# MicahZoltu/lodestar

Measured on AMD Instinct MI355X. Metric: verified signature sets/sec (mainnet attestation mix), higher is better.
Workload: dtype u32 (381-bit Montgomery; device products on 14x28-bit limbs); 1 GPU; c3: gossip attestation flood, 6 slot(s) per batch, 7 batches in flight per GPU; slots_per_batch=6, sets_per_gpu=116736, jobs_per_gpu=104448, pubkeys_per_gpu=1683456, parallelism=dp1 (sets sharded), exchange=False, inflight=7, world_size_seen=1, pubkeys=indices into the GPU-resident table, signing_roots_per_gpu=6918

## Files before the change

lodestar_amd/csrc/lb_consts.h:

```cpp
#pragma once
#include "lb_common.h"

#define LB_PINV 0xfffcfffdu
#define LB_X_ABS 0xd201000000010000ull
#define LB_PINV28 0xffcfffdu
#define LB_P28_0 0xfffaaabu
#define LB_P28_1 0xfefffffu
#define LB_P28_2 0x3ffffb9u
#define LB_P28_3 0xfffeb15u
#define LB_P28_4 0x6241eabu
#define LB_P28_5 0xa0f6b0fu
#define LB_P28_6 0xf6730d2u
#define LB_P28_7 0xf38512bu
#define LB_P28_8 0x4774b84u
#define LB_P28_9 0x4bacd76u
#define LB_P28_10 0xba7b643u
#define LB_P28_11 0xe69a4b1u
#define LB_P28_12 0x1ea397fu
#define LB_P28_13 0x001a011u
#define LB_P0 0xffffaaabu
#define LB_P1 0xb9feffffu
#define LB_P2 0xb153ffffu
#define LB_P3 0x1eabfffeu
#define LB_P4 0xf6b0f624u
#define LB_P5 0x6730d2a0u
#define LB_P6 0xf38512bfu
#define LB_P7 0x64774b84u
#define LB_P8 0x434bacd7u
#define LB_P9 0x4b1ba7b6u
#define LB_P10 0x397fe69au
#define LB_P11 0x1a0111eau
LB_CONST uint32_t LB_P[12] = {0xffffaaab, 0xb9feffff, 0xb153ffff, 0x1eabfffe, 0xf6b0f624, 0x6730d2a0, 0xf38512bf, 0x64774b84, 0x434bacd7, 0x4b1ba7b6, 0x397fe69a, 0x1a0111ea};
LB_CONST uint32_t LB_ONE[12] = {0x0002fffd, 0x76090000, 0xc40c0002, 0xebf4000b, 0x53c758ba, 0x5f489857, 0x70525745, 0x77ce5853, 0xa256ec6d, 0x5c071a97, 0xfa80e493, 0x15f65ec3};
LB_CONST uint32_t LB_R2[12] = {0x1c341746, 0xf4df1f34, 0x09d104f1, 0x0a76e6a6, 0x4c95b6d5, 0x8de5476c, 0x939d83c0, 0x67eb88a9, 0xb519952d, 0x9a793e85, 0x92cae3aa, 0x11988fe5};
LB_CONST uint32_t LB_2P256[12] = {0xc5ce820f, 0x075b3cd7, 0x1c3edb0b, 0x3ec6ba62, 0x2bff6bce, 0x168a13d8, 0xf8c449d2, 0x87663c4b, 0xddc8d830, 0x15f34c83, 0x9caa2e85, 0x0f9628b4};
LB_CONST uint32_t LB_B1[12] = {0x000cfff3, 0xaa270000, 0xfc34000a, 0x53cc0032, 0x6b0a807f, 0x478fe97a, 0xe6ba24d7, 0xb1d37ebe, 0xbf78ab2f, 0x8ec9733b, 0x3d83de7e, 0x09d64551};
LB_CONST uint32_t LB_B1_3[12] = {0x0027552e, 0x44760000, 0x43480020, 0xdcb8009a, 0x4a6e8b59, 0x6f7ee9ce, 0xc0a95bc6, 0xb10330b7, 0xfb1e54b7, 0x6140b1fc, 0x7f0bb4e1, 0x0381be09};
LB_CONST uint32_t LB_B2[24] = {0x000cfff3, 0xaa270000, 0xfc34000a, 0x53cc0032, 0x6b0a807f, 0x478fe97a, 0xe6ba24d7, 0xb1d37ebe, 0xbf78ab2f, 0x8ec9733b, 0x3d83de7e, 0x09d64551, 0x000cfff3, 0xaa270000, 0xfc34000a, 0x53cc0032, 0x6b0a807f, 0x478fe97a, 0xe6ba24d7, 0xb1d37ebe, 0xbf78ab2f, 0x8ec9733b, 0x3d83de7e, 0x09d64551};
LB_CONST uint32_t LB_B2_3[24] = {0x0027552e, 0x44760000, 0x43480020, 0xdcb8009a, 0x4a6e8b59, 0x6f7ee9ce, 0xc0a95bc6, 0xb10330b7, 0xfb1e54b7, 0x6140b1fc, 0x7f0bb4e1, 0x0381be09, 0x0027552e, 0x44760000, 0x43480020, 0xdcb8009a, 0x4a6e8b59, 0x6f7ee9ce, 0xc0a95bc6, 0xb10330b7, 0xfb1e54b7, 0x6140b1fc, 0x7f0bb4e1, 0x0381be09};
LB_CONST uint32_t LB_EXP_PM2[12] = {0xffffaaa9, 0xb9feffff, 0xb153ffff, 0x1eabfffe, 0xf6b0f624, 0x6730d2a0, 0xf38512bf, 0x64774b84, 0x434bacd7, 0x4b1ba7b6, 0x397fe69a, 0x1a0111ea};
LB_CONST uint32_t LB_EXP_SQRT[12] = {0xffffeaab, 0xee7fbfff, 0xac54ffff, 0x07aaffff, 0x3dac3d89, 0xd9cc34a8, 0x3ce144af, 0xd91dd2e1, 0x90d2eb35, 0x92c6e9ed, 0x8e5ff9a6, 0x0680447a};
LB_CONST uint32_t LB_EXP_ISQRT[12] = {0xffffeaaa, 0xee7fbfff, 0xac54ffff, 0x07aaffff, 0x3dac3d89, 0xd9cc34a8, 0x3ce144af, 0xd91dd2e1, 0x90d2eb35, 0x92c6e9ed, 0x8e5ff9a6, 0x0680447a};
LB_CONST uint32_t LB_EXP_LEGENDRE[12] = {0xffffd555, 0xdcff7fff, 0x58a9ffff, 0x0f55ffff, 0x7b587b12, 0xb3986950, 0x79c2895f, 0xb23ba5c2, 0x21a5d66b, 0x258dd3db, 0x1cbff34d, 0x0d0088f5};
LB_CONST uint32_t LB_HALF_P[12] = {0xffffd555, 0xdcff7fff, 0x58a9ffff, 0x0f55ffff, 0x7b587b12, 0xb3986950, 0x79c2895f, 0xb23ba5c2, 0x21a5d66b, 0x258dd3db, 0x1cbff34d, 0x0d0088f5};
LB_CONST uint32_t LB_INV2[12] = {0x00015554, 0x18040000, 0x3ab00001, 0x85500005, 0x253c276f, 0x633cb57c, 0x31ebb502, 0x6e22d1ec, 0xf2d14ca2, 0xd3916126, 0x1a006596, 0x17fbb857};
LB_CONST uint32_t LB_R3[12] = {0xd94ca1e0, 0xed48ac6b, 0x03a7adf8, 0x315f831e, 0x615e29dd, 0x9a53352a, 0x921e1761, 0x34c04e5e, 0x65724728, 0x2512d435, 0x91755d4d, 0x0aa63460};
LB_CONST uint32_t LB_P_X1[13] = {0xffffaaab, 0xb9feffff, 0xb153ffff, 0x1eabfffe, 0xf6b0f624, 0x6730d2a0, 0xf38512bf, 0x64774b84, 0x434bacd7, 0x4b1ba7b6, 0x397fe69a, 0x1a0111ea, 0x00000000};
LB_CONST uint32_t LB_P_X2[13] = {0xffff5556, 0x73fdffff, 0x62a7ffff, 0x3d57fffd, 0xed61ec48, 0xce61a541, 0xe70a257e, 0xc8ee9709, 0x869759ae, 0x96374f6c, 0x72ffcd34, 0x340223d4, 0x00000000};
LB_CONST uint32_t LB_P_X4[13] = {0xfffeaaac, 0xe7fbffff, 0xc54ffffe, 0x7aaffffa, 0xdac3d890, 0x9cc34a83, 0xce144afd, 0x91dd2e13, 0x0d2eb35d, 0x2c6e9ed9, 0xe5ff9a69, 0x680447a8, 0x00000000};
LB_CONST uint32_t LB_P_X8[13] = {0xfffd5558, 0xcff7ffff, 0x8a9ffffd, 0xf55ffff5, 0xb587b120, 0x39869507, 0x9c2895fb, 0x23ba5c27, 0x1a5d66bb, 0x58dd3db2, 0xcbff34d2, 0xd0088f51, 0x00000000};
LB_CONST uint32_t LB_P_X16[13] = {0xfffaaab0, 0x9fefffff, 0x153ffffb, 0xeabfffeb, 0x6b0f6241, 0x730d2a0f, 0x38512bf6, 0x4774b84f, 0x34bacd76, 0xb1ba7b64, 0x97fe69a4, 0xa0111ea3, 0x00000001};
LB_CONST uint32_t LB_P_X32[13] = {0xfff55560, 0x3fdfffff, 0x2a7ffff7, 0xd57fffd6, 0xd61ec483, 0xe61a541e, 0x70a257ec, 0x8ee9709e, 0x69759aec, 0x6374f6c8, 0x2ffcd349, 0x40223d47, 0x00000003};
// ... 43 lines not shown
```

lodestar_amd/csrc/lb_curve.h:

```cpp
#pragma once
#include "lb_field.h"

template <class F>
struct jac {
  F x, y, z;
};
template <class F>
struct aff {
  F x, y;
};

typedef jac<fp> g1j;
typedef jac<fp2> g2j;
typedef aff<fp> g1a;
typedef aff<fp2> g2a;

template <class T, class S>
LB_HD aff<T> aff_as(const aff<S>& a) {
  return aff<T>{T{a.x}, T{a.y}};
}
template <class T, class S>
LB_HD jac<T> jac_as(const jac<S>& a) {
  return jac<T>{T{a.x}, T{a.y}, T{a.z}};
}
// ... 343 lines not shown
  p.y = fp2_sub(lean2_mul<kInl>(rr, fp2_sub(V, p.x)), YJ);
}

template <bool kInl>
LB_HD void g2_add_lean(g2j& p, const g2j& q) {
  if (jac_is_inf(q)) return;
  if (jac_is_inf(p)) {
    p = q;
    return;
  }
  const fp2 Z1Z1 = lean2_sqr<kInl>(p.z), Z2Z2 = lean2_sqr<kInl>(q.z);
  const fp2 ZZ = fp2_sub(fp2_sub(lean2_sqr<kInl>(fp2_add(p.z, q.z)), Z1Z1), Z2Z2);
  const fp2 U1 = lean2_mul<kInl>(p.x, Z2Z2);
  const fp2 S1 = lean2_mul<kInl>(lean2_mul<kInl>(p.y, q.z), Z2Z2);
  const fp2 H = fp2_sub(lean2_mul<kInl>(q.x, Z1Z1), U1);
  const fp2 rr = fp2_dbl(fp2_sub(lean2_mul<kInl>(lean2_mul<kInl>(q.y, p.z), Z1Z1), S1));
  if (fp2_is_zero(H)) {
    if (fp2_is_zero(rr)) {
      p = q;
      g2_dbl_lean<kInl>(p);
    } else {
      p = jac_infinity<fp2>();
    }
    return;
  }
  p.z = lean2_mul<kInl>(ZZ, H);
  const fp2 I = lean2_sqr<kInl>(fp2_dbl(H));
  const fp2 J = lean2_mul<kInl>(H, I);
  const fp2 V = lean2_mul<kInl>(U1, I);
  p.x = fp2_sub(fp2_sub(lean2_sqr<kInl>(rr), J), fp2_dbl(V));
  p.y = fp2_sub(lean2_mul<kInl>(rr, fp2_sub(V, p.x)), fp2_dbl(lean2_mul<kInl>(S1, J)));
}

LB_HD bool g2_aff_in_subgroup_i(const g2a& a) {
  g2j acc = jac_from_aff(a);
#pragma clang loop unroll(disable)
  for (int i = 62; i >= 0; i--) {
    acc = jac_dbl_i(acc);
    if ((LB_X_ABS >> i) & 1ull) acc = jac_add_aff_i<fp2, true>(acc, a);
  }
  if (jac_is_inf(acc)) return false;
  fp2 z2 = fp2_sqr(acc.z);
  fp2 px = fp2_mul(fp2_conj(a.x), fp2_load(LB_PSI_CX));
  if (!fp2_eq(fp2_mul(px, z2), acc.x)) return false;
  fp2 py = fp2_mul(fp2_conj(a.y), fp2_load(LB_PSI_CY));
  return fp2_eq(fp2_mul(fp2_mul(py, z2), acc.z), fp2_neg(acc.y));
}

LB_NI g2j g2_clear_cofactor(g2j p) {
  g2j t1 = jac_neg(jac_mul_xabs(p));
  g2j t2 = g2_psi(p);
  g2j t3 = g2_psi2(jac_dbl(p));
  t3 = jac_add(t3, jac_neg(t2));
  t2 = jac_add(t1, t2);
  t2 = jac_neg(jac_mul_xabs(t2));
  t3 = jac_add(t3, t2);
  t3 = jac_add(t3, jac_neg(t1));
  return jac_add(t3, jac_neg(p));
}

LB_HD bool g1_aff_on_curve(const g1a& a) {
  return fp_eq(fp_sqr(a.y), fp_add(fp_mul(fp_sqr(a.x), a.x), fp_load(LB_B1)));
}
LB_HD bool g2_aff_on_curve(const g2a& a) {
  return fp2_eq(fp2_sqr(a.y), fp2_add(fp2_mul(fp2_sqr(a.x), a.x), fp2_load(LB_B2)));
}
// ... 1 lines not shown
```

lodestar_amd/csrc/lb_field.h:

```cpp
#pragma once
#include "lb_common.h"
#include "lb_consts.h"

struct fp {
  uint32_t v[12];
};
struct fp2 {
  fp c0, c1;
};
struct fp6 {
  fp2 c0, c1, c2;
};
struct fp12 {
  fp6 c0, c1;
};

LB_HD fp fp_load(const uint32_t* c) {
  fp r;
  LB_UNROLL for (int i = 0; i < 12; i++) r.v[i] = c[i];
  return r;
}
LB_HD fp2 fp2_load(const uint32_t* c) {
  fp2 r;
  r.c0 = fp_load(c);
// ... 231 lines not shown

LB_HD fp lb_tab8(const fp* t, uint32_t k) {
  switch (k) {
    case 0: return t[0];
    case 1: return t[1];
    case 2: return t[2];
    case 3: return t[3];
    case 4: return t[4];
    case 5: return t[5];
    case 6: return t[6];
    default: return t[7];
  }
}
LB_HD fp fp_mul_inl(const fp& a, const fp& b) {
#if defined(__HIP_DEVICE_COMPILE__)
  __builtin_amdgcn_sched_barrier(0);
  const fp r = fp_mul28(a, b);
  __builtin_amdgcn_sched_barrier(0);
  return r;
#else
  return fp_mul(a, b);
#endif
}
LB_HD fp fp_sqr_inl(const fp& a) {
#if defined(__HIP_DEVICE_COMPILE__)
  __builtin_amdgcn_sched_barrier(0);
  const fp r = fp_sqr28(a);
  __builtin_amdgcn_sched_barrier(0);
  return r;
#else
  return fp_sqr(a);
#endif
}
struct fp28 {
  uint32_t l[14];
};
LB_HD fp28 fp28_mul_raw(const fp28& a, const fp28& b) {
  const uint32_t P28[14] = {LB_P28_0, LB_P28_1, LB_P28_2, LB_P28_3, LB_P28_4,  LB_P28_5,  LB_P28_6,
                            LB_P28_7, LB_P28_8, LB_P28_9, LB_P28_10, LB_P28_11, LB_P28_12, LB_P28_13};
  uint64_t acc[28];
  LB_UNROLL for (int k = 0; k < 28; k++) acc[k] = 0;
  LB_UNROLL for (int i = 0; i < 14; i++) {
    LB_UNROLL for (int j = 0; j < 14; j++) acc[i + j] += (uint64_t)a.l[i] * b.l[j];
    const uint32_t m = ((uint32_t)acc[i] * LB_PINV28) & 0x0fffffffu;
    LB_UNROLL for (int j = 0; j < 14; j++) acc[i + j] += (uint64_t)m * P28[j];
    acc[i + 1] += acc[i] >> 28;
  }
  fp28 r;
  LB_UNROLL for (int k = 0; k < 13; k++) {
    r.l[k] = (uint32_t)acc[14 + k] & 0x0fffffffu;
    acc[15 + k] += acc[14 + k] >> 28;
  }
  r.l[13] = (uint32_t)acc[27];
  return r;
}
LB_HD fp28 fp28_sqr_raw(const fp28& a) {
  const uint32_t P28[14] = {LB_P28_0, LB_P28_1, LB_P28_2, LB_P28_3, LB_P28_4,  LB_P28_5,  LB_P28_6,
                            LB_P28_7, LB_P28_8, LB_P28_9, LB_P28_10, LB_P28_11, LB_P28_12, LB_P28_13};
  uint32_t D[14];
  LB_UNROLL for (int k = 0; k < 14; k++) D[k] = a.l[k] << 1;
  uint64_t acc[28];
  LB_UNROLL for (int k = 0; k < 28; k++) acc[k] = 0;
  LB_UNROLL for (int i = 0; i < 14; i++) {
    acc[2 * i] += (uint64_t)a.l[i] * a.l[i];
    LB_UNROLL for (int j = i + 1; j < 14; j++) acc[i + j] += (uint64_t)D[i] * a.l[j];
  }
  LB_UNROLL for (int i = 0; i < 14; i++) {
    const uint32_t m = ((uint32_t)acc[i] * LB_PINV28) & 0x0fffffffu;
    LB_UNROLL for (int j = 0; j < 14; j++) acc[i + j] += (uint64_t)m * P28[j];
    acc[i + 1] += acc[i] >> 28;
  }
  fp28 r;
  LB_UNROLL for (int k = 0; k < 13; k++) {
    r.l[k] = (uint32_t)acc[14 + k] & 0x0fffffffu;
    acc[15 + k] += acc[14 + k] >> 28;
  }
  r.l[13] = (uint32_t)acc[27];
  return r;
}
LB_HD fp28 fp28_mul(const fp28& a, const fp28& b) {
#if defined(__HIP_DEVICE_COMPILE__)
  __builtin_amdgcn_sched_barrier(0);
  const fp28 r = fp28_mul_raw(a, b);
  __builtin_amdgcn_sched_barrier(0);
  return r;
#else
  return fp28_mul_raw(a, b);
#endif
}
LB_HD fp28 fp28_sqr(const fp28& a) {
#if defined(__HIP_DEVICE_COMPILE__)
  __builtin_amdgcn_sched_barrier(0);
  const fp28 r = fp28_sqr_raw(a);
  __builtin_amdgcn_sched_barrier(0);
  return r;
#else
  return fp28_sqr_raw(a);
#endif
}
LB_HD fp28 lb_tab8_28(const fp28* t, uint32_t k) {
  switch (k) {
    case 0: return t[0];
    case 1: return t[1];
    case 2: return t[2];
    case 3: return t[3];
    case 4: return t[4];
    case 5: return t[5];
    case 6: return t[6];
    default: return t[7];
// ... 10 lines not shown
  fp28 r = tab[0];
  bool first = true;
  int i = top_bit;
  while (i >= 0) {
    if (!bit(i)) {
      if (!first) r = fp28_sqr(r);
      i--;
      continue;
    }
    int j = i - (WIN - 1) > 0 ? i - (WIN - 1) : 0;
    while (!bit(j)) j++;
    uint32_t val = 0;
    for (int k = i; k >= j; k--) val = (val << 1) | bit(k);
    if (first) {
      r = lb_tab8_28(tab, val >> 1);
      first = false;
    } else {
      for (int k = i; k >= j; k--) r = fp28_sqr(r);
      r = fp28_mul(r, lb_tab8_28(tab, val >> 1));
    }
    i = j - 1;
  }
  const fp one = fp_one();
  fp28 c;
  LB_UNROLL for (int k = 0; k < 14; k++) c.l[k] = lb_bits28(one.v, 28 * k);
  const fp28 t = fp28_mul(r, c);
  uint32_t o[12];
  LB_UNROLL for (int w = 0; w < 12; w++) {
    const int l = (32 * w) / 28, s = 32 * w - 28 * l;
    o[w] = (t.l[l] >> s) | (t.l[l + 1] << (28 - s));
  }
  return fp_reduce_once(o, 0u);
}

template <bool kInlMul = false>
LB_HD fp fp_pow_const_i(fp a, const uint32_t* e, int top_bit) {
  if constexpr (kInlMul) return fp_pow_const_28(a, e, top_bit);
  fp tab[8];
  tab[0] = a;
  const fp a2 = fp_sqr(a);
  LB_UNROLL for (int k = 1; k < 8; k++) tab[k] = fp_mul(tab[k - 1], a2);
  auto bit = [&](int i) -> uint32_t { return (e[i >> 5] >> (i & 31)) & 1u; };
  fp r = fp_zero();
  bool first = true;
  int i = top_bit;
  while (i >= 0) {
    if (!bit(i)) {
      r = fp_sqr(r);
      i--;
      continue;
    }
    int j = i - 3 > 0 ? i - 3 : 0;
    while (!bit(j)) j++;
    uint32_t val = 0;
    for (int k = i; k >= j; k--) val = (val << 1) | bit(k);
    if (first) {
      r = lb_tab8(tab, val >> 1);
      first = false;
    } else {
      for (int k = i; k >= j; k--) r = fp_sqr(r);
      r = fp_mul(r, lb_tab8(tab, val >> 1));
    }
    i = j - 1;
  }
  return r;
}
// ... 605 lines not shown
```

lodestar_amd/csrc/lb_kernels.h:

```cpp
#pragma once
#include "lb_serial.h"
#include "lb_h2c.h"
#include "lb_pairing.h"

#define LB_TPB 64
#ifndef LB_MINW
#define LB_MINW 1
#endif
#ifndef LB_MINW_DEC
#define LB_MINW_DEC 2
#endif
#ifndef LB_MINW_SUB
#define LB_MINW_SUB LB_MINW_DEC
#endif
#ifndef LB_MINW_MSM
#define LB_MINW_MSM 1
#endif
#ifndef LB_MINW_GSUM
#define LB_MINW_GSUM 1
#endif
typedef fpi lb_g1f;
typedef fp2i lb_g2f;
typedef jac<lb_g2f> g2jm;
#ifndef LB_MINW_G1
// ... 118 lines not shown
  int st = LB_OK;
  g2a a;
  bool inf = false;
  if (sig_sizes != nullptr && sig_sizes[i] != 96) {
    st = LB_INVALID_SIZE;
    a.x = fp2_zero();
    a.y = fp2_zero();
  } else {
    uint32_t w[24];
    const uint4* s = reinterpret_cast<const uint4*>(sigs + (size_t)96 * i);
    LB_UNROLL for (int k = 0; k < 6; k++) {
      const uint4 v = s[k];
      w[4 * k] = v.x, w[4 * k + 1] = v.y, w[4 * k + 2] = v.z, w[4 * k + 3] = v.w;
    }
    st = g2_decompress96_w(w, a, inf);
  }
  soa_st(sig_aff, n, i, a);
  const uint32_t* w = reinterpret_cast<const uint32_t*>(&a);
  LB_UNROLL for (int k = 0; k < 12; k++) sig_aos[(size_t)12 * i + k] = make_uint4(w[4 * k], w[4 * k + 1], w[4 * k + 2], w[4 * k + 3]);
  sig_inf[i] = inf ? 1u : 0u;
  sig_status[i] = st;
}
#endif

#if LB_KG(1)
__global__ void __launch_bounds__(LB_TPB, LB_MINW_SUB) k_sig_subgroup(uint32_t n, const uint32_t* __restrict__ sig_aff,
                                                         const uint32_t* __restrict__ sig_inf,
                                                         int32_t* __restrict__ sig_status) {
  uint32_t i = lb_tid();
  if (i >= n) return;
  if (sig_status[i] != LB_OK || sig_inf[i]) return;
  auto load_f2 = [&](int o) {
    const uint32_t* base = sig_aff;
    asm volatile("" : "+s"(base));
    fp2 a;
    uint32_t* w = reinterpret_cast<uint32_t*>(&a);
    LB_UNROLL for (int k = 0; k < 24; k++) w[k] = __builtin_nontemporal_load(base + (size_t)(k + o) * n + i);
    return a;
  };
  g2j acc = jac_from_aff(g2a{load_f2(0), load_f2(24)});
  bool redo = false;
#pragma clang loop unroll(disable)
  for (int b = 62; b >= 0;) {
    g2_dbl_lean<true>(acc);
    if (redo) {
      redo = false;
      b--;
      continue;
    }
    if ((LB_X_ABS >> b) & 1ull) {
      if (jac_is_inf(acc)) {
        acc = jac_from_aff(g2a{load_f2(0), load_f2(24)});
        b--;
        continue;
      }
      const fp2 Z1Z1 = lean2_sqr<true>(acc.z);
      const fp2 H = fp2_sub(lean2_mul<true>(load_f2(0), Z1Z1), acc.x);
      const fp2 t = lean2_mul<true>(acc.z, Z1Z1);
      const fp2 rr = fp2_dbl(fp2_sub(lean2_mul<true>(load_f2(24), t), acc.y));
      if (fp2_is_zero(H)) {
        if (fp2_is_zero(rr)) {
          acc = jac_from_aff(g2a{load_f2(0), load_f2(24)});
          redo = true;
        } else {
          acc = jac_infinity<fp2>();
          b--;
        }
        continue;
      }
      acc.z = fp2_dbl(lean2_mul<true>(acc.z, H));
      const fp2 I = fp2_mul4(lean2_sqr<true>(H));
      const fp2 J = lean2_mul<true>(H, I);
      const fp2 V = lean2_mul<true>(acc.x, I);
      const fp2 YJ = fp2_dbl(lean2_mul<true>(acc.y, J));
      acc.x = fp2_sub(fp2_sub(lean2_sqr<true>(rr), J), fp2_dbl(V));
      acc.y = fp2_sub(lean2_mul<true>(rr, fp2_sub(V, acc.x)), YJ);
    }
    b--;
  }
  bool ok = !jac_is_inf(acc);
  if (ok) {
    const fp2 z2 = lean2_sqr<true>(acc.z);
    ok = fp2_eq(lean2_mul<true>(lean2_mul<true>(fp2_conj(load_f2(0)), fp2_load(LB_PSI_CX)), z2),
                acc.x);
    if (ok) {
      const fp2 py = lean2_mul<true>(fp2_conj(load_f2(24)), fp2_load(LB_PSI_CY));
      ok = fp2_eq(lean2_mul<true>(lean2_mul<true>(py, z2), acc.z), fp2_neg(acc.y));
    }
  }
  if (!ok) sig_status[i] = LB_POINT_NOT_IN_GROUP;
}
#endif

#if LB_KG(1)
__global__ void __launch_bounds__(64) k_sig_subgroup_g8(uint32_t n, const uint32_t* __restrict__ sig_aff,
                                                        const uint32_t* __restrict__ sig_inf,
                                                        int32_t* __restrict__ sig_status) {
  __shared__ uint32_t g8s[8 * 72];
  const uint32_t i = blockIdx.x * 8 + (threadIdx.x >> 3);
  if (i >= n) return;
  if (sig_status[i] != LB_OK || sig_inf[i]) return;
  lds_u32* G = (lds_u32*)g8s + (threadIdx.x >> 3) * 72;
  g8_stash(G, 0, jac_from_aff(soa_ld<g2a>(sig_aff, n, i)));
  const g2j acc = g8_mul_xabs_st(G, 0);
  bool ok = !jac_is_inf(acc);
  if (ok) ok = jac_eq(g8_psi(g8_unstash(G, 0)), jac_neg(acc));
  if (!ok && g8_q() == 0) sig_status[i] = LB_POINT_NOT_IN_GROUP;
}
#endif

typedef uint32_t lb_v8u __attribute__((ext_vector_type(8)));
static __device__ __attribute__((noinline)) lb_v8u sha256_compress_v(lb_v8u hv, lb_v16u bv) {
  uint32_t h[8], blk[16];
  LB_UNROLL for (int i = 0; i < 8; i++) h[i] = hv[i];
  LB_UNROLL for (int i = 0; i < 16; i++) blk[i] = bv[i];
  sha256_compress(h, blk);
  lb_v8u r;
  LB_UNROLL for (int i = 0; i < 8; i++) r[i] = h[i];
  return r;
}
__device__ __forceinline__ uint32_t dst_byte(int k) { return k < LB_DST_LEN + 1 ? (uint32_t)LB_DST[k] : 0u; }
__device__ __forceinline__ uint32_t dst_word(int k) {
// ... 2427 lines not shown
```

Before: 11.91 million sets/s.

## Run G2 subgroup check in lazy-reduced 28-bit limb representation

Rewrites the signature subgroup-check kernel so the x-multiplication loop runs entirely in a 14x28-bit limb representation. Additions and subtractions are lazy, with offset constants and explicit normalisation, and fp2 products use fused two-product Montgomery accumulation (mac2). One intermediate is parked in LDS to reduce register pressure. It also adds an optional host-side bound-checking mode that tracks limb bounds to validate the lazy-reduction headroom. This trades more intricate bound reasoning, and the risk of overflow if the bounds are wrong, for fewer full reductions and conversions per point operation.

```diff
diff --git a/lodestar_amd/csrc/lb_consts.h b/lodestar_amd/csrc/lb_consts.h
--- a/lodestar_amd/csrc/lb_consts.h
+++ b/lodestar_amd/csrc/lb_consts.h
@@ -18,6 +18,34 @@
 #define LB_P28_11 0xe69a4b1u
 #define LB_P28_12 0x1ea397fu
 #define LB_P28_13 0x001a011u
+#define LB_R28_ONE_0 0x347fcb8u
+#define LB_R28_ONE_1 0xd800000u
+#define LB_R28_ONE_2 0x002b119u
+#define LB_R28_ONE_3 0x0cde6d2u
+#define LB_R28_ONE_4 0xc7212e0u
+#define LB_R28_ONE_5 0x83a2090u
+#define LB_R28_ONE_6 0x037669fu
+#define LB_R28_ONE_7 0xda0f73eu
+#define LB_R28_ONE_8 0x9b09b42u
+#define LB_R28_ONE_9 0x1297bb0u
+#define LB_R28_ONE_10 0x515d98fu
+#define LB_R28_ONE_11 0x012ca7cu
+#define LB_R28_ONE_12 0x659fcfau
+#define LB_R28_ONE_13 0x000577au
+#define LB_R28_IN_0 0x80e6299u
+#define LB_R28_IN_1 0x3500034u
+#define LB_R28_IN_2 0xeb12856u
+#define LB_R28_IN_3 0xdeb2699u
+#define LB_R28_IN_4 0xc988670u
+#define LB_R28_IN_5 0x4ef6697u
+#define LB_R28_IN_6 0x70983e8u
+#define LB_R28_IN_7 0xa4e6fe9u
+#define LB_R28_IN_8 0x3e8a053u
+#define LB_R28_IN_9 0xecf271eu
+#define LB_R28_IN_10 0xc20d323u
+#define LB_R28_IN_11 0x6eb6385u
+#define LB_R28_IN_12 0x47f1286u
+#define LB_R28_IN_13 0x00156dau
 #define LB_P0 0xffffaaabu
 #define LB_P1 0xb9feffffu
 #define LB_P2 0xb153ffffu
diff --git a/lodestar_amd/csrc/lb_curve.h b/lodestar_amd/csrc/lb_curve.h
--- a/lodestar_amd/csrc/lb_curve.h
+++ b/lodestar_amd/csrc/lb_curve.h
@@ -399,6 +399,121 @@
   p.y = fp2_sub(lean2_mul<kInl>(rr, fp2_sub(V, p.x)), fp2_dbl(lean2_mul<kInl>(S1, J)));
 }
 
+#define LB_L28_VX 30.0
+#define LB_L28_VY 12.0
+#define LB_L28_VZ 3.0
+struct g2j28 {
+  fp2_28 x, y, z;
+};
+#if defined(LB_FP28_CHECK)
+static inline void fp28_chk_assume(fp28& a, double vb) {
+  for (int k = 0; k < 13; k++) LB_CHK_ASSERT(a.ub[k] <= 0x0fffffffu);
+  LB_CHK_ASSERT(a.vb <= vb && a.ub[13] <= fp28_chk_top(vb));
+  fp28_chk_set(a, vb);
+}
+static inline void g2j28_chk_assume(g2j28& p) {
+  fp28_chk_assume(p.x.c0, LB_L28_VX), fp28_chk_assume(p.x.c1, LB_L28_VX);
+  fp28_chk_assume(p.y.c0, LB_L28_VY), fp28_chk_assume(p.y.c1, LB_L28_VY);
+  fp28_chk_assume(p.z.c0, LB_L28_VZ), fp28_chk_assume(p.z.c1, LB_L28_VZ);
+}
+#endif
+LB_HD g2j28 g2j28_from_aff(const fp2& x, const fp2& y) {
+  return g2j28{fp2_28_from_fp2(x), fp2_28_from_fp2(y), fp2_28{fp28_one(), fp28_zero()}};
+}
+LB_HD g2j28 g2j28_infinity() {
+  return g2j28{fp2_28{fp28_one(), fp28_zero()}, fp2_28{fp28_one(), fp28_zero()}, fp2_28{fp28_zero(), fp28_zero()}};
+}
+LB_HD bool g2j28_is_inf(const g2j28& p) { return fp2_28_is_zero(p.z); }
+LB_HD g2j g2j28_to_g2j(const g2j28& p) {
+  g2j r;
+  r.x = fp2_28_to_fp2(p.x);
+  r.y = fp2_28_to_fp2(p.y);
+  r.z = fp2_28_to_fp2(p.z);
+  return r;
+}
+LB_HD void g2_dbl_lean28(g2j28& p) {
+  LB_CHK(g2j28_chk_assume(p);)
+  p.z = fp2_28_norm(fp2_28_muls<2>(fp2_28_mul<13, 28>(p.z, p.y)));
+  const fp2_28 B = fp2_28_sqr<13, 28>(p.y);
+  const fp2_28 C = fp2_28_sqr<2, 28>(B);
+  const fp2_28 A = fp2_28_sqr<31, 28>(p.x);
+  fp2_28 D = fp2_28_sqr<32, 28>(fp2_28_norm(fp2_28_add(p.x, B)));
+  D = fp2_28_norm(fp2_28_muls<2>(fp2_28_sub<4, 29>(D, fp2_28_add(A, C))));
+  const fp2_28 E = fp2_28_norm(fp2_28_muls<3>(A));
+  p.x = fp2_28_norm(fp2_28_sub<27, 29>(fp2_28_sqr<8, 28>(E), fp2_28_muls<2>(D)));
+  p.y = fp2_28_norm(fp2_28_sub<9, 31>(fp2_28_mul<8, 28>(fp2_28_sub<29, 28>(D, p.x), E),
+                                      fp2_28_muls<8>(C)));
+}
+#if defined(__HIPCC__)
+#define LB_HDM __host__ __device__ __forceinline__
+#else
+#define LB_HDM inline
+#endif
+struct g2_park28 {
+  fp2_28 v;
+  LB_HDM void put(const fp2_28& a) { v = a; }
+  LB_HDM fp2_28 get() const { return v; }
+};
+template <class Ld, class Pk>
+LB_HD int g2_madd_lean28(g2j28& p, Ld&& ld, Pk&& pk) {
+  LB_CHK(g2j28_chk_assume(p);)
+  pk.put(p.y);
+  const fp2_28 Z1Z1 = fp2_28_sqr<4, 28>(p.z);
+  const fp2_28 H = fp2_28_norm(fp2_28_sub<31, 28>(fp2_28_mul<2, 28>(fp2_28_from_fp2_shift(ld(0)), Z1Z1), p.x));
+  const fp2_28 t = fp2_28_mul<2, 28>(p.z, Z1Z1);
+  const fp2_28 S2 = fp2_28_mul<2, 28>(fp2_28_from_fp2_shift(ld(24)), t);
+  const fp2_28 rr = fp2_28_norm(fp2_28_muls<2>(fp2_28_sub<13, 28>(S2, pk.get())));
+  if (fp2_28_is_zero(H)) return fp2_28_is_zero(rr) ? 1 : 2;
+  p.z = fp2_28_norm(fp2_28_muls<2>(fp2_28_mul<4, 28>(H, p.z)));
+  const fp2_28 I = fp2_28_muls<4>(fp2_28_sqr<33, 28>(H));
+  const fp2_28 J = fp2_28_mul<33, 28>(I, H);
+  const fp2_28 V = fp2_28_mul<31, 28>(I, p.x);
+  pk.put(fp2_28_muls<2>(fp2_28_mul<2, 28>(pk.get(), J)));
+  p.x = fp2_28_norm(fp2_28_sub<5, 30>(fp2_28_sqr<29, 28>(rr), fp2_28_add(J, fp2_28_muls<2>(V))));
+  const fp2_28 Y3 = fp2_28_mul<29, 28>(fp2_28_sub<8, 28>(V, p.x), rr);
+  p.y = fp2_28_norm(fp2_28_sub<3, 29>(Y3, pk.get()));
+  return 0;
+}
+template <class Ld, class Pk>
+LB_HD bool g2_aff_in_subgroup28(Ld&& ld, Pk&& pk) {
+  g2j28 acc = g2j28_from_aff(ld(0), ld(24));
+  bool redo = false;
+#pragma clang loop unroll(disable)
+  for (int b = 62; b >= 0;) {
+    g2_dbl_lean28(acc);
+    if (redo) {
+      redo = false;
+      b--;
+      continue;
+    }
+    if ((LB_X_ABS >> b) & 1ull) {
+      if (g2j28_is_inf(acc)) {
+        acc = g2j28_from_aff(ld(0), ld(24));
+        b--;
+        continue;
+      }
+      const int e = g2_madd_lean28(acc, ld, pk);
+      if (e == 1) {
+        acc = g2j28_from_aff(ld(0), ld(24));
+        redo = true;
+        continue;
+      }
+      if (e == 2) {
+        acc = g2j28_infinity();
+        b--;
+        continue;
+      }
+    }
+    b--;
+  }
+  if (g2j28_is_inf(acc)) return false;
+  const g2j a = g2j28_to_g2j(acc);
+  const fp2 z2 = lean2_sqr<true>(a.z);
+  if (!fp2_eq(lean2_mul<true>(lean2_mul<true>(fp2_conj(ld(0)), fp2_load(LB_PSI_CX)), z2), a.x)) return false;
+  const fp2 py = lean2_mul<true>(fp2_conj(ld(24)), fp2_load(LB_PSI_CY));
+  return fp2_eq(lean2_mul<true>(lean2_mul<true>(py, z2), a.z), fp2_neg(a.y));
+}
+
 LB_HD bool g2_aff_in_subgroup_i(const g2a& a) {
   g2j acc = jac_from_aff(a);
 #pragma clang loop unroll(disable)
diff --git a/lodestar_amd/csrc/lb_field.h b/lodestar_amd/csrc/lb_field.h
--- a/lodestar_amd/csrc/lb_field.h
+++ b/lodestar_amd/csrc/lb_field.h
@@ -287,8 +287,27 @@
   return fp_sqr(a);
 #endif
 }
+#if defined(LB_FP28_CHECK)
+#include <stdio.h>
+#include <stdlib.h>
+#define LB_CHK(...) __VA_ARGS__
+#define LB_CHK_ASSERT(c)                                                                \
+  do {                                                                                  \
+    if (!(c)) {                                                                         \
+      fprintf(stderr, "fp28 bound violated: %s (%s:%d)\n", #c, __FILE__, __LINE__);     \
+      abort();                                                                          \
+    }                                                                                   \
+  } while (0)
+#define LB_COL_CHK(acc, x, y) \
+  LB_CHK_ASSERT((unsigned __int128)(acc) + (unsigned __int128)(x) * (y) <= (unsigned __int128)~0ull)
+#else
+#define LB_CHK(...)
+#define LB_CHK_ASSERT(c) ((void)0)
+#define LB_COL_CHK(acc, x, y) ((void)0)
+#endif
 struct fp28 {
   uint32_t l[14];
+  LB_CHK(uint64_t ub[14]; double vb;)
 };
 LB_HD fp28 fp28_mul_raw(const fp28& a, const fp28& b) {
   const uint32_t P28[14] = {LB_P28_0, LB_P28_1, LB_P28_2, LB_P28_3, LB_P28_4,  LB_P28_5,  LB_P28_6,
@@ -296,16 +315,25 @@
   uint64_t acc[28];
   LB_UNROLL for (int k = 0; k < 28; k++) acc[k] = 0;
   LB_UNROLL for (int i = 0; i < 14; i++) {
-    LB_UNROLL for (int j = 0; j < 14; j++) acc[i + j] += (uint64_t)a.l[i] * b.l[j];
+    LB_UNROLL for (int j = 0; j < 14; j++) {
+      LB_COL_CHK(acc[i + j], a.l[i], b.l[j]);
+      acc[i + j] += (uint64_t)a.l[i] * b.l[j];
+    }
     const uint32_t m = ((uint32_t)acc[i] * LB_PINV28) & 0x0fffffffu;
-    LB_UNROLL for (int j = 0; j < 14; j++) acc[i + j] += (uint64_t)m * P28[j];
+    LB_UNROLL for (int j = 0; j < 14; j++) {
+      LB_COL_CHK(acc[i + j], m, P28[j]);
+      acc[i + j] += (uint64_t)m * P28[j];
+    }
+    LB_COL_CHK(acc[i + 1], acc[i] >> 28, 1u);
     acc[i + 1] += acc[i] >> 28;
   }
   fp28 r;
   LB_UNROLL for (int k = 0; k < 13; k++) {
     r.l[k] = (uint32_t)acc[14 + k] & 0x0fffffffu;
+    LB_COL_CHK(acc[15 + k], acc[14 + k] >> 28, 1u);
     acc[15 + k] += acc[14 + k] >> 28;
   }
+  LB_CHK_ASSERT(acc[27] < (1ull << 28));
   r.l[13] = (uint32_t)acc[27];
   return r;
 }
@@ -317,19 +345,30 @@
   uint64_t acc[28];
   LB_UNROLL for (int k = 0; k < 28; k++) acc[k] = 0;
   LB_UNROLL for (int i = 0; i < 14; i++) {
+    LB_CHK_ASSERT(a.l[i] < (1u << 31));
+    LB_COL_CHK(acc[2 * i], a.l[i], a.l[i]);
     acc[2 * i] += (uint64_t)a.l[i] * a.l[i];
-    LB_UNROLL for (int j = i + 1; j < 14; j++) acc[i + j] += (uint64_t)D[i] * a.l[j];
+    LB_UNROLL for (int j = i + 1; j < 14; j++) {
+      LB_COL_CHK(acc[i + j], D[i], a.l[j]);
+      acc[i + j] += (uint64_t)D[i] * a.l[j];
+    }
   }
   LB_UNROLL for (int i = 0; i < 14; i++) {
     const uint32_t m = ((uint32_t)acc[i] * LB_PINV28) & 0x0fffffffu;
-    LB_UNROLL for (int j = 0; j < 14; j++) acc[i + j] += (uint64_t)m * P28[j];
+    LB_UNROLL for (int j = 0; j < 14; j++) {
+      LB_COL_CHK(acc[i + j], m, P28[j]);
+      acc[i + j] += (uint64_t)m * P28[j];
+    }
+    LB_COL_CHK(acc[i + 1], acc[i] >> 28, 1u);
     acc[i + 1] += acc[i] >> 28;
   }
   fp28 r;
   LB_UNROLL for (int k = 0; k < 13; k++) {
     r.l[k] = (uint32_t)acc[14 + k] & 0x0fffffffu;
+    LB_COL_CHK(acc[15 + k], acc[14 + k] >> 28, 1u);
     acc[15 + k] += acc[14 + k] >> 28;
   }
+  LB_CHK_ASSERT(acc[27] < (1ull << 28));
   r.l[13] = (uint32_t)acc[27];
   return r;
 }
@@ -406,6 +445,264 @@
   }
   return fp_reduce_once(o, 0u);
 }
+
+LB_HD constexpr uint32_t lb_k28_limb(uint32_t c, int s, int i) {
+  const uint32_t P28[14] = {LB_P28_0, LB_P28_1, LB_P28_2, LB_P28_3, LB_P28_4,  LB_P28_5,  LB_P28_6,
+                            LB_P28_7, LB_P28_8, LB_P28_9, LB_P28_10, LB_P28_11, LB_P28_12, LB_P28_13};
+  uint64_t carry = 0, k = 0;
+  for (int j = 0; j <= i; j++) {
+    const uint64_t t = (uint64_t)c * P28[j] + carry;
+    k = j < 13 ? (t & 0x0fffffffu) : t;
+    carry = t >> 28;
+  }
+  const uint64_t b = 1ull << s, bh = 1ull << (s - 28);
+  return (uint32_t)(i == 0 ? k + b : i < 13 ? k + b - bh : k - bh);
+}
+#define LB_K28(C, S)                                                                                          \
+  {lb_k28_limb(C, S, 0), lb_k28_limb(C, S, 1), lb_k28_limb(C, S, 2),  lb_k28_limb(C, S, 3),  lb_k28_limb(C, S, 4), \
+   lb_k28_limb(C, S, 5), lb_k28_limb(C, S, 6), lb_k28_limb(C, S, 7),  lb_k28_limb(C, S, 8),  lb_k28_limb(C, S, 9), \
+   lb_k28_limb(C, S, 10), lb_k28_limb(C, S, 11), lb_k28_limb(C, S, 12), lb_k28_limb(C, S, 13)}
+
+#if defined(LB_FP28_CHECK)
+static inline uint64_t fp28_chk_top(double vb) { return (uint64_t)(vb * 106513.2) + 1; }
+static inline void fp28_chk_set(fp28& a, double vb) {
+  for (int k = 0; k < 13; k++) a.ub[k] = 0x0fffffffu;
+  a.ub[13] = fp28_chk_top(vb) < 0x0fffffffu ? fp28_chk_top(vb) : 0x0fffffffu;
+  a.vb = vb;
+}
+static inline void fp28_chk_in(const fp28& a) {
+  for (int k = 0; k < 14; k++) LB_CHK_ASSERT(a.l[k] <= a.ub[k]);
+}
+static inline void fp28_chk_mac(const fp28& a, const fp28& b, const fp28* c, const fp28* d, fp28& r) {
+  const uint32_t P28[14] = {LB_P28_0, LB_P28_1, LB_P28_2, LB_P28_3, LB_P28_4,  LB_P28_5,  LB_P28_6,
+                            LB_P28_7, LB_P28_8, LB_P28_9, LB_P28_10, LB_P28_11, LB_P28_12, LB_P28_13};
+  typedef unsigned __int128 u128;
+  const u128 lim = (u128)~0ull;
+  fp28_chk_in(a), fp28_chk_in(b);
+  if (c) fp28_chk_in(*c), fp28_chk_in(*d);
+  u128 col[29];
+  for (int k = 0; k < 29; k++) col[k] = 0;
+  for (int i = 0; i < 14; i++) {
+    for (int j = 0; j < 14; j++) {
+      col[i + j] += (u128)a.ub[i] * b.ub[j] + (u128)0x0fffffffu * P28[j];
+      if (c) col[i + j] += (u128)c->ub[i] * d->ub[j];
+    }
+    LB_CHK_ASSERT(col[i] <= lim);
+    col[i + 1] += col[i] >> 28;
+  }
+  for (int k = 14; k < 28; k++) {
+    LB_CHK_ASSERT(col[k] <= lim);
+    col[k + 1] += col[k] >> 28;
+  }
+  const double s = a.vb * b.vb + (c ? c->vb * d->vb : 0.0);
+  const double vb = (1.0 + s / 2520.0) * (1.0 + 1e-9);
+  LB_CHK_ASSERT(vb < 2520.0);
+  fp28_chk_set(r, vb);
+}
+#endif
+
+struct fp2_28 {
+  fp28 c0, c1;
+};
+LB_HD fp28 fp28_add(const fp28& a, const fp28& b) {
+  fp28 r;
+  LB_UNROLL for (int k = 0; k < 14; k++) {
+    r.l[k] = a.l[k] + b.l[k];
+    LB_CHK(r.ub[k] = a.ub[k] + b.ub[k]; LB_CHK_ASSERT(r.ub[k] <= 0xffffffffull);)
+  }
+  LB_CHK(r.vb = a.vb + b.vb;)
+  return r;
+}
+template <int N>
+LB_HD fp28 fp28_muls(const fp28& a) {
+  fp28 r;
+  LB_UNROLL for (int k = 0; k < 14; k++) {
+    r.l[k] = N == 3 ? (a.l[k] << 1) + a.l[k] : a.l[k] << (N == 2 ? 1 : N == 4 ? 2 : 3);
+    LB_CHK(r.ub[k] = N * a.ub[k]; LB_CHK_ASSERT(r.ub[k] <= 0xffffffffull);)
+  }
+  LB_CHK(r.vb = N * a.vb;)
+  return r;
+}
+template <uint32_t C, int S>
+LB_HD fp28 fp28_kminus(const fp28& b) {
+  constexpr uint32_t K[14] = LB_K28(C, S);
+  fp28 r;
+  LB_UNROLL for (int k = 0; k < 14; k++) {
+    r.l[k] = K[k] - b.l[k];
+    LB_CHK(LB_CHK_ASSERT(b.ub[k] <= K[k]); r.ub[k] = K[k];)
+  }
+  LB_CHK(r.vb = C;)
+  return r;
+}
+template <uint32_t C, int S>
+LB_HD fp28 fp28_sub(const fp28& a, const fp28& b) {
+  constexpr uint32_t K[14] = LB_K28(C, S);
+  fp28 r;
+  LB_UNROLL for (int k = 0; k < 14; k++) {
+    r.l[k] = a.l[k] + K[k] - b.l[k];
+    LB_CHK(LB_CHK_ASSERT(b.ub[k] <= K[k]); r.ub[k] = a.ub[k] + K[k]; LB_CHK_ASSERT(r.ub[k] <= 0xffffffffull);)
+  }
+  LB_CHK(r.vb = a.vb + C;)
+  return r;
+}
+LB_HD fp28 fp28_norm(const fp28& a) {
+  fp28 r;
+  uint32_t c = 0;
+  LB_CHK(uint64_t cb = 0;)
+  LB_UNROLL for (int k = 0; k < 13; k++) {
+    const uint32_t t = a.l[k] + c;
+    LB_CHK(LB_CHK_ASSERT(a.ub[k] + cb <= 0xffffffffull); cb = (a.ub[k] + cb) >> 28;)
+    r.l[k] = t & 0x0fffffffu;
+    c = t >> 28;
+  }
+  r.l[13] = a.l[13] + c;
+  LB_CHK(const uint64_t top = a.ub[13] + cb; fp28_chk_set(r, a.vb); if (top < r.ub[13]) r.ub[13] = top;)
+  return r;
+}
+LB_HD fp28 fp28_mulx(const fp28& a, const fp28& b) {
+#if defined(__HIP_DEVICE_COMPILE__)
+  __builtin_amdgcn_sched_barrier(0);
+#endif
+  fp28 r = fp28_mul_raw(a, b);
+#if defined(__HIP_DEVICE_COMPILE__)
+  __builtin_amdgcn_sched_barrier(0);
+#endif
+  LB_CHK(fp28_chk_mac(a, b, nullptr, nullptr, r);)
+  return r;
+}
+LB_HD fp28 fp28_mac2(const fp28& a, const fp28& b, const fp28& c, const fp28& d) {
+  const uint32_t P28[14] = {LB_P28_0, LB_P28_1, LB_P28_2, LB_P28_3, LB_P28_4,  LB_P28_5,  LB_P28_6,
+                            LB_P28_7, LB_P28_8, LB_P28_9, LB_P28_10, LB_P28_11, LB_P28_12, LB_P28_13};
+#if defined(__HIP_DEVICE_COMPILE__)
+  __builtin_amdgcn_sched_barrier(0);
+#endif
+  uint64_t acc[28];
+  LB_UNROLL for (int k = 0; k < 28; k++) acc[k] = 0;
+  LB_UNROLL for (int i = 0; i < 14; i++) {
+    LB_UNROLL for (int j = 0; j < 14; j++) {
+      LB_COL_CHK(acc[i + j], a.l[i], b.l[j]);
+      acc[i + j] += (uint64_t)a.l[i] * b.l[j];
+    }
+    LB_UNROLL for (int j = 0; j < 14; j++) {
+      LB_COL_CHK(acc[i + j], c.l[i], d.l[j]);
+      acc[i + j] += (uint64_t)c.l[i] * d.l[j];
+    }
+    const uint32_t m = ((uint32_t)acc[i] * LB_PINV28) & 0x0fffffffu;
+    LB_UNROLL for (int j = 0; j < 14; j++) {
+      LB_COL_CHK(acc[i + j], m, P28[j]);
+      acc[i + j] += (uint64_t)m * P28[j];
+    }
+    LB_COL_CHK(acc[i + 1], acc[i] >> 28, 1u);
+    acc[i + 1] += acc[i] >> 28;
+  }
+  fp28 r;
+  LB_UNROLL for (int k = 0; k < 13; k++) {
+    r.l[k] = (uint32_t)acc[14 + k] & 0x0fffffffu;
+    LB_COL_CHK(acc[15 + k], acc[14 + k] >> 28, 1u);
+    acc[15 + k] += acc[14 + k] >> 28;
+  }
+  LB_CHK_ASSERT(acc[27] < (1ull << 28));
+  r.l[13] = (uint32_t)acc[27];
+#if defined(__HIP_DEVICE_COMPILE__)
+  __builtin_amdgcn_sched_barrier(0);
+#endif
+  LB_CHK(fp28_chk_mac(a, b, &c, &d, r);)
+  return r;
+}
+
+LB_HD fp28 fp28_one() {
+  const uint32_t c[14] = {LB_R28_ONE_0, LB_R28_ONE_1, LB_R28_ONE_2, LB_R28_ONE_3, LB_R28_ONE_4,  LB_R28_ONE_5,  LB_R28_ONE_6,
+                          LB_R28_ONE_7, LB_R28_ONE_8, LB_R28_ONE_9, LB_R28_ONE_10, LB_R28_ONE_11, LB_R28_ONE_12, LB_R28_ONE_13};
+  fp28 r;
+  LB_UNROLL for (int k = 0; k < 14; k++) r.l[k] = c[k];
+  LB_CHK(fp28_chk_set(r, 1.0);)
+  return r;
+}
+LB_HD fp28 fp28_zero() {
+  fp28 r;
+  LB_UNROLL for (int k = 0; k < 14; k++) r.l[k] = 0;
+  LB_CHK(fp28_chk_set(r, 1.0);)
+  return r;
+}
+LB_HD fp28 fp28_from_fp_shift(const fp& a) {
+  fp28 r;
+  r.l[0] = (a.v[0] << 8) & 0x0fffffffu;
+  LB_UNROLL for (int k = 1; k < 14; k++) r.l[k] = lb_bits28(a.v, 28 * k - 8);
+  LB_CHK(fp28_chk_set(r, 256.0);)
+  return r;
+}
+LB_HD fp28 fp28_from_fp(const fp& a) {
+  const uint32_t c[14] = {LB_R28_IN_0, LB_R28_IN_1, LB_R28_IN_2, LB_R28_IN_3, LB_R28_IN_4,  LB_R28_IN_5,  LB_R28_IN_6,
+                          LB_R28_IN_7, LB_R28_IN_8, LB_R28_IN_9, LB_R28_IN_10, LB_R28_IN_11, LB_R28_IN_12, LB_R28_IN_13};
+  fp28 x, k;
+  LB_UNROLL for (int i = 0; i < 14; i++) x.l[i] = lb_bits28(a.v, 28 * i), k.l[i] = c[i];
+  LB_CHK(fp28_chk_set(x, 1.0); fp28_chk_set(k, 1.0);)
+  return fp28_mulx(x, k);
+}
+LB_HD fp fp28_to_fp(const fp28& a) {
+  const fp one = fp_one();
+  fp28 c;
+  LB_UNROLL for (int k = 0; k < 14; k++) c.l[k] = lb_bits28(one.v, 28 * k);
+  LB_CHK(fp28_chk_set(c, 1.0);)
+  const fp28 t = fp28_mulx(a, c);
+  LB_CHK_ASSERT(t.vb < 2.0);
+  uint32_t o[12];
+  LB_UNROLL for (int w = 0; w < 12; w++) {
+    const int l = (32 * w) / 28, s = 32 * w - 28 * l;
+    o[w] = (t.l[l] >> s) | (t.l[l + 1] << (28 - s));
+  }
+  return fp_reduce_once(o, 0u);
+}
+LB_HD bool fp28_is_zero(const fp28& a) {
+  const uint32_t P28[14] = {LB_P28_0, LB_P28_1, LB_P28_2, LB_P28_3, LB_P28_4,  LB_P28_5,  LB_P28_6,
+                            LB_P28_7, LB_P28_8, LB_P28_9, LB_P28_10, LB_P28_11, LB_P28_12, LB_P28_13};
+  LB_CHK(fp28_chk_in(a); LB_CHK_ASSERT(a.vb < 2520.0);)
+  uint64_t acc[28];
+  LB_UNROLL for (int k = 0; k < 28; k++) acc[k] = k < 14 ? a.l[k] : 0;
+  LB_UNROLL for (int i = 0; i < 14; i++) {
+    const uint32_t m = ((uint32_t)acc[i] * LB_PINV28) & 0x0fffffffu;
+    LB_UNROLL for (int j = 0; j < 14; j++) acc[i + j] += (uint64_t)m * P28[j];
+    acc[i + 1] += acc[i] >> 28;
+  }
+  uint32_t z = 0, e = 0;
+  LB_UNROLL for (int k = 0; k < 14; k++) {
+    const uint32_t t = k < 13 ? ((uint32_t)acc[14 + k] & 0x0fffffffu) : (uint32_t)acc[27];
+    if (k < 13) acc[15 + k] += acc[14 + k] >> 28;
+    z |= t;
+    e |= t ^ P28[k];
+  }
+  return z == 0 || e == 0;
+}
+
+LB_HD fp2_28 fp2_28_add(const fp2_28& a, const fp2_28& b) { return fp2_28{fp28_add(a.c0, b.c0), fp28_add(a.c1, b.c1)}; }
+template <int N>
+LB_HD fp2_28 fp2_28_muls(const fp2_28& a) {
+  return fp2_28{fp28_muls<N>(a.c0), fp28_muls<N>(a.c1)};
+}
+template <uint32_t C, int S>
+LB_HD fp2_28 fp2_28_sub(const fp2_28& a, const fp2_28& b) {
+  return fp2_28{fp28_sub<C, S>(a.c0, b.c0), fp28_sub<C, S>(a.c1, b.c1)};
+}
+LB_HD fp2_28 fp2_28_norm(const fp2_28& a) { return fp2_28{fp28_norm(a.c0), fp28_norm(a.c1)}; }
+template <uint32_t C, int S>
+LB_HD fp2_28 fp2_28_mul(const fp2_28& a, const fp2_28& b) {
+  const fp28 nb1 = fp28_kminus<C, S>(b.c1);
+  fp2_28 r;
+  r.c0 = fp28_mac2(a.c0, b.c0, a.c1, nb1);
+  r.c1 = fp28_mac2(a.c0, b.c1, a.c1, b.c0);
+  return r;
+}
+template <uint32_t C, int S>
+LB_HD fp2_28 fp2_28_sqr(const fp2_28& a) {
+  fp2_28 r;
+  r.c0 = fp28_mulx(fp28_add(a.c0, a.c1), fp28_sub<C, S>(a.c0, a.c1));
+  r.c1 = fp28_mulx(fp28_muls<2>(a.c0), a.c1);
+  return r;
+}
+LB_HD bool fp2_28_is_zero(const fp2_28& a) { return fp28_is_zero(a.c0) & fp28_is_zero(a.c1); }
+LB_HD fp2_28 fp2_28_from_fp2(const fp2& a) { return fp2_28{fp28_from_fp(a.c0), fp28_from_fp(a.c1)}; }
+LB_HD fp2_28 fp2_28_from_fp2_shift(const fp2& a) { return fp2_28{fp28_from_fp_shift(a.c0), fp28_from_fp_shift(a.c1)}; }
+LB_HD fp2 fp2_28_to_fp2(const fp2_28& a) { return fp2{fp28_to_fp(a.c0), fp28_to_fp(a.c1)}; }
 
 template <bool kInlMul = false>
 LB_HD fp fp_pow_const_i(fp a, const uint32_t* e, int top_bit) {
diff --git a/lodestar_amd/csrc/lb_kernels.h b/lodestar_amd/csrc/lb_kernels.h
--- a/lodestar_amd/csrc/lb_kernels.h
+++ b/lodestar_amd/csrc/lb_kernels.h
@@ -174,62 +174,27 @@
   if (sig_status[i] != LB_OK || sig_inf[i]) return;
   auto load_f2 = [&](int o) {
     const uint32_t* base = sig_aff;
-    asm volatile("" : "+s"(base));
+    uint32_t l = i;
+    asm volatile("" : "+s"(base), "+v"(l));
     fp2 a;
     uint32_t* w = reinterpret_cast<uint32_t*>(&a);
-    LB_UNROLL for (int k = 0; k < 24; k++) w[k] = __builtin_nontemporal_load(base + (size_t)(k + o) * n + i);
+    LB_UNROLL for (int k = 0; k < 24; k++) w[k] = __builtin_nontemporal_load(base + (size_t)(k + o) * n + l);
     return a;
   };
-  g2j acc = jac_from_aff(g2a{load_f2(0), load_f2(24)});
-  bool redo = false;
-#pragma clang loop unroll(disable)
-  for (int b = 62; b >= 0;) {
-    g2_dbl_lean<true>(acc);
-    if (redo) {
-      redo = false;
-      b--;
-      continue;
-    }
-    if ((LB_X_ABS >> b) & 1ull) {
-      if (jac_is_inf(acc)) {
-        acc = jac_from_aff(g2a{load_f2(0), load_f2(24)});
-        b--;
-        continue;
-      }
-      const fp2 Z1Z1 = lean2_sqr<true>(acc.z);
-      const fp2 H = fp2_sub(lean2_mul<true>(load_f2(0), Z1Z1), acc.x);
-      const fp2 t = lean2_mul<true>(acc.z, Z1Z1);
-      const fp2 rr = fp2_dbl(fp2_sub(lean2_mul<true>(load_f2(24), t), acc.y));
-      if (fp2_is_zero(H)) {
-        if (fp2_is_zero(rr)) {
-          acc = jac_from_aff(g2a{load_f2(0), load_f2(24)});
-          redo = true;
-        } else {
-          acc = jac_infinity<fp2>();
-          b--;
-        }
-        continue;
-      }
-      acc.z = fp2_dbl(lean2_mul<true>(acc.z, H));
-      const fp2 I = fp2_mul4(lean2_sqr<true>(H));
-      const fp2 J = lean2_mul<true>(H, I);
-      const fp2 V = lean2_mul<true>(acc.x, I);
-      const fp2 YJ = fp2_dbl(lean2_mul<true>(acc.y, J));
-      acc.x = fp2_sub(fp2_sub(lean2_sqr<true>(rr), J), fp2_dbl(V));
-      acc.y = fp2_sub(lean2_mul<true>(rr, fp2_sub(V, acc.x)), YJ);
-    }
-    b--;
-  }
-  bool ok = !jac_is_inf(acc);
-  if (ok) {
-    const fp2 z2 = lean2_sqr<true>(acc.z);
-    ok = fp2_eq(lean2_mul<true>(lean2_mul<true>(fp2_conj(load_f2(0)), fp2_load(LB_PSI_CX)), z2),
-                acc.x);
-    if (ok) {
-      const fp2 py = lean2_mul<true>(fp2_conj(load_f2(24)), fp2_load(LB_PSI_CY));
-      ok = fp2_eq(lean2_mul<true>(lean2_mul<true>(py, z2), acc.z), fp2_neg(acc.y));
-    }
-  }
+  __shared__ uint32_t park[28 * LB_TPB];
+  struct {
+    uint32_t* s;
+    __device__ __forceinline__ void put(const fp2_28& a) {
+      LB_UNROLL for (int k = 0; k < 14; k++) s[LB_TPB * k] = a.c0.l[k], s[LB_TPB * (14 + k)] = a.c1.l[k];
+    }
+    __device__ __forceinline__ fp2_28 get() const {
+      fp2_28 a;
+      LB_UNROLL for (int k = 0; k < 14; k++) a.c0.l[k] = s[LB_TPB * k], a.c1.l[k] = s[LB_TPB * (14 + k)];
+      return a;
+    }
+  } pk{park + threadIdx.x};
+  const bool ok = g2_aff_in_subgroup28(load_f2, pk);
+  asm volatile("" : "+v"(i));
   if (!ok) sig_status[i] = LB_POINT_NOT_IN_GROUP;
 }
 #endif
```

Result: faster. 12.16 million sets/s (median of 6 runs) (+2.1%).
